# Kang-ChangWoo/audio-depth-estimation

Hardware: AMD Instinct MI355X
Metric: depth-maps/sec (train step) (higher is better)
Workload: dtype bf16; 1 GPU; unetbaseline_model unet_256 (ngf 64) train step, BatVisionV2-shaped 256x256, batch 32/GPU, Combined L1+SIlog loss, clip 1.0, AdamW; global_batch=32, image_size=256, launch=hipGraph, parallelism=dp1

## Files before the change

### audio-depth-estimation_amd/_lib.py

```python
from __future__ import annotations

import ctypes as C
import os

_HERE = os.path.dirname(os.path.abspath(__file__))
LIB_PATH = os.environ.get('ADN_LIB', os.path.join(_HERE, 'libadn.so'))

ADN_F32, ADN_BF16 = 0, 1
GEMM_S2, GEMM_T2, GEMM_S1 = 0, 1, 2
EPI_RAW, EPI_Z_STATS, EPI_ACT, EPI_BWD, EPI_FINAL, EPI_ADD = 0, 1, 2, 3, 4, 5

c_void_p, c_int32, c_int64, c_float = C.c_void_p, C.c_int32, C.c_int64, C.c_float


class AdnEpiSeg(C.Structure):
    _fields_ = [
        ('out0', c_void_p), ('out1', c_void_p), ('ref', c_void_p), ('z', c_void_p),
        ('mean', c_void_p), ('istd', c_void_p), ('scale', c_void_p), ('shift', c_void_p),
        ('bias', c_void_p), ('partials', c_void_p),
        ('channels', c_int32), ('slope', c_float), ('accumulate', c_int32), ('final_act', c_int32),
    ]


class AdnIgemmDesc(C.Structure):
    _fields_ = [
        ('dtype', c_int32), ('geom', c_int32), ('B', c_int32), ('Hs', c_int32), ('Ws', c_int32),
        ('C0', c_int32), ('C1', c_int32), ('N', c_int32),
        ('in0', c_void_p), ('in1', c_void_p), ('w', c_void_p),
        ('epi', c_int32), ('seg', AdnEpiSeg * 2),
        ('workspace', c_void_p), ('workspace_bytes', c_int64),
        ('ks', c_int32), ('reserved', c_int32),
    ]


class AdnMx8ConvDesc(C.Structure):
    _fields_ = [
        ('B', c_int32), ('H', c_int32), ('W', c_int32), ('C0', c_int32), ('C1', c_int32), ('N', c_int32),
        ('in0', c_void_p), ('sc0', c_void_p), ('in1', c_void_p), ('sc1', c_void_p), ('w', c_void_p), ('wsc', c_void_p),
        ('epi', c_int32), ('reserved', c_int32), ('seg', AdnEpiSeg * 2),
    ]


class AdnWgradDesc(C.Structure):
    _fields_ = [
        ('dtype', c_int32), ('B', c_int32), ('Hs', c_int32), ('Ws', c_int32),
        ('plain0', c_void_p), ('plain1', c_void_p), ('R0', c_int32), ('R1', c_int32),
        ('gath0', c_void_p), ('gath1', c_void_p), ('C0', c_int32), ('C1', c_int32),
        ('dw', c_void_p), ('workspace', c_void_p), ('workspace_bytes', c_int64), ('c_valid', c_int32),
        ('geom', c_int32), ('ks', c_int32), ('sq_partials', c_void_p),
    ]


class AdnAttnDesc(C.Structure):
    _fields_ = [
        ('dtype', c_int32), ('B2', c_int32), ('N', c_int32), ('dqk', c_int32), ('dv', c_int32), ('kv_shift', c_int32),
        ('q', c_void_p), ('k', c_void_p), ('v', c_void_p),
        ('ld_q', c_int32), ('ld_k', c_int32), ('ld_v', c_int32),
        ('o', c_void_p), ('ld_o', c_int32),
        ('lse', c_void_p), ('scale', c_float),
        ('dout', c_void_p), ('ld_do', c_int32),
        ('dq', c_void_p), ('dk', c_void_p), ('dvp', c_void_p),
        ('ld_dq', c_int32), ('ld_dk', c_int32), ('ld_dv', c_int32),
        ('workspace', c_void_p), ('workspace_bytes', c_int64),
    ]


class AdnDistillSmall(C.Structure):
    _fields_ = [
        ('mean_student', c_void_p), ('mean_teacher', c_void_p), ('centers_student', c_void_p), ('centers_teacher', c_void_p),
        ('feat_stats', c_void_p * 5), ('feat_channels', c_int32 * 5),
        ('pix_stats', c_void_p),
        ('B', c_int32), ('nb', c_int32), ('has_teacher', c_int32),
        ('temperature', c_float), ('lambda_task', c_float), ('lambda_response', c_float), ('lambda_feature', c_float),
        ('lambda_bin', c_float), ('lambda_sparse', c_float),
        ('terms', c_void_p), ('dmean', c_void_p), ('dcent', c_void_p),
    ]


class AdnCoarseLoss(C.Structure):
    _fields_ = [
        ('logits', c_void_p), ('dtype', c_int32), ('nb', c_int32), ('ld', c_int32), ('ce_mode', c_int32),
        ('pixels', c_int64), ('pixels_global', c_int64),
        ('centers', c_void_p), ('bins', c_void_p), ('gt', c_void_p), ('n_valid', c_void_p),
        ('sigma', c_float), ('gamma', c_float), ('ce_weight', c_float), ('reg_weight', c_float),
        ('depth', c_void_p), ('argmax', c_void_p), ('dlogits', c_void_p),
        ('workspace', c_void_p), ('workspace_bytes', c_int64),
    ]


class AdnDualRegLoss(C.Structure):
    _fields_ = [
        ('coarse', c_void_p), ('offset', c_void_p), ('gt', c_void_p), ('n_valid', c_void_p),
        ('pixels', c_int64), ('pixels_global', c_int64),
        ('coarse_weight', c_float), ('final_weight', c_float), ('offset_reg_weight', c_float),
        ('final_depth', c_void_p), ('dcoarse', c_void_p), ('doffset', c_void_p),
        ('workspace', c_void_p), ('workspace_bytes', c_int64),
    ]


class AdnHybridLoss(C.Structure):
    _fields_ = [
        ('logits', c_void_p), ('dtype', c_int32), ('nb', c_int32), ('ld', c_int32), ('reg_mode', c_int32),
        ('pixels', c_int64), ('pixels_global', c_int64),
        ('centers', c_void_p), ('coarse', c_void_p), ('offset', c_void_p), ('bins', c_void_p), ('gt', c_void_p),
        ('ce_weight', c_float), ('reg_weight', c_float), ('offset_reg_weight', c_float), ('label_smoothing', c_float),
        ('final_depth', c_void_p), ('dlogits', c_void_p), ('doffset', c_void_p),
        ('workspace', c_void_p), ('workspace_bytes', c_int64),
    ]


_PROTOS = {
    'adn_last_error': (C.c_char_p, []),
    'adn_version': (C.c_int, []),
    'adn_debug_poison_lds': (C.c_int, [c_void_p]),
    'adn_debug_stream_rmw': (C.c_int, [c_void_p, c_void_p, c_int64, c_int32, c_int32, c_void_p]),
    'adn_igemm_num_partials': (c_int64, [C.POINTER(AdnIgemmDesc)]),
    'adn_igemm_workspace_bytes': (c_int64, [C.POINTER(AdnIgemmDesc)]),
    'adn_igemm_describe': (C.c_int, [C.POINTER(AdnIgemmDesc), C.c_char_p, C.c_int]),
    'adn_igemm': (C.c_int, [C.POINTER(AdnIgemmDesc), c_void_p]),
    'adn_wgrad_workspace_bytes': (c_int64, [C.POINTER(AdnWgradDesc)]),
    'adn_wgrad': (C.c_int, [C.POINTER(AdnWgradDesc), c_void_p]),
    'adn_wgrad_batchable': (c_int32, [C.POINTER(AdnWgradDesc)]),
    'adn_wgrad_batch_sq_count': (c_int32, [C.POINTER(AdnWgradDesc)]),
    'adn_wgrad_batch': (C.c_int, [C.POINTER(AdnWgradDesc), c_int32, c_void_p]),
    'adn_wgrad_multi': (C.c_int, [C.POINTER(AdnWgradDesc), c_int32, c_void_p]),
    'adn_wgrad_patch_batch_workspace_bytes': (c_int64, [C.POINTER(AdnWgradDesc), c_int32]),
    'adn_wgrad_patch_batch': (C.c_int, [C.POINTER(AdnWgradDesc), c_int32, c_void_p]),
    'adn_wgrad_sq_count': (c_int32, [C.POINTER(AdnWgradDesc)]),
    'adn_pack_weights': (C.c_int, [c_void_p, c_int32, c_int32, c_int32, c_int32, c_void_p, c_void_p, c_void_p]),
    'adn_mx8_quantize': (C.c_int, [c_void_p, c_int64, c_int32, c_void_p, c_void_p, c_void_p]),
    'adn_mx8_pack': (C.c_int, [c_void_p, c_int32, c_int32, c_int32, c_void_p, c_void_p, c_void_p]),
    'adn_bn_partials_reduce': (C.c_int, [c_void_p, c_int64, c_int32, c_int32, c_void_p, c_void_p]),
    'adn_tail_stats_blocks': (c_int64, [c_int64, c_int32]),
    'adn_maxpool2_bwd_tail': (C.c_int, [c_void_p, c_void_p, c_void_p, c_int32, c_int32, c_int32, c_int32, c_int32, c_int32, c_void_p,
                                        c_void_p, c_void_p, c_void_p, c_void_p]),
    'adn_upsample2x_bwd_tail': (C.c_int, [c_void_p, c_void_p, c_int32, c_int32, c_int32, c_int32, c_int32, c_int32, c_int32, c_int32,
                                          c_void_p, c_void_p, c_void_p, c_void_p, c_void_p, c_void_p]),
    'adn_maxpool2_fwd_mx8': (C.c_int, [c_void_p, c_void_p, c_int32, c_int32, c_int32, c_int32, c_void_p, c_void_p, c_void_p]),
    'adn_upsample2x_fwd_mx8': (C.c_int, [c_void_p, c_void_p, c_int32, c_int32, c_int32, c_int32, c_int32, c_int32, c_void_p,
                                         c_void_p, c_void_p]),
    'adn_bn_act_mx8': (C.c_int, [c_void_p, c_int64, c_int32, c_void_p, c_void_p, c_void_p, c_void_p, c_void_p, c_void_p]),
    'adn_bn_bwd_apply_mx8': (C.c_int, [c_void_p, c_void_p, c_int64, c_int32, c_void_p, c_void_p, c_void_p, c_void_p, c_void_p,
                                       c_void_p, c_void_p]),
    'adn_conv3x3_mx8_num_partials': (c_int64, [C.POINTER(AdnMx8ConvDesc)]),
    'adn_conv3x3_mx8': (C.c_int, [C.POINTER(AdnMx8ConvDesc), c_void_p]),
    'adn_pack_rows': (C.c_int, [c_void_p, c_int32, c_int32, c_int32, c_int32, c_int32, c_int32, c_void_p, c_void_p]),
    'adn_pack_transpose_taps': (C.c_int, [c_void_p, c_int32, c_int32, c_int32, c_int32, c_int32, c_int32, c_void_p,
                                          c_void_p]),
    'adn_maxpool2_fwd': (C.c_int, [c_void_p, c_void_p, c_int32, c_int32, c_int32, c_int32, c_int32, c_void_p]),
    'adn_maxpool2_bwd': (C.c_int, [c_void_p, c_void_p, c_void_p, c_int32, c_int32, c_int32, c_int32, c_int32, c_int32, c_void_p]),
    'adn_upsample2x_fwd': (C.c_int, [c_void_p, c_void_p, c_int32, c_int32, c_int32, c_int32, c_int32, c_int32, c_int32, c_void_p]),
    'adn_upsample2x_bwd': (C.c_int, [c_void_p, c_void_p, c_int32, c_int32, c_int32, c_int32, c_int32, c_int32, c_int32, c_int32, c_void_p]),
    'adn_pixel_shuffle2': (C.c_int, [c_void_p, c_void_p, c_int32, c_int32, c_int32, c_int32, c_int32, c_int32, c_void_p]),
    'adn_relu_bwd_stats_num_partials': (c_int64, [c_int64, c_int32]),
    'adn_relu_bwd_stats': (C.c_int, [c_void_p, c_void_p, c_void_p, c_void_p, c_void_p, c_int64, c_int32, c_int32, c_void_p, c_void_p]),
    'adn_head1x1_fwd': (C.c_int, [c_void_p, c_void_p, c_void_p, c_int64, c_int32, c_int32, c_int32, c_float, c_void_p, c_void_p, c_void_p]),
    'adn_head1x1_bwd_workspace_bytes': (c_int64, [c_int64, c_int32]),
    'adn_head1x1_bwd': (C.c_int, [c_void_p, c_void_p, c_void_p, c_void_p, c_int64, c_int32, c_int32, c_int32, c_float, c_void_p, c_void_p, c_void_p, c_void_p,
                                  c_int64, c_void_p]),
    'adn_l1tv_workspace_bytes': (c_int64, [c_int64]),
    'adn_l1tv_stats': (C.c_int, [c_void_p, c_void_p, c_int32, c_int32, c_int32, c_void_p, c_void_p, c_int64, c_void_p]),
    'adn_l1tv_finish': (C.c_int, [c_void_p, c_void_p, c_int32, c_int32, c_int32, c_void_p, c_int32, c_float, c_float, c_void_p, c_void_p, c_void_p]),
    'adn_nchw_to_nhwc': (C.c_int, [c_void_p, c_void_p, c_int32, c_int32, c_int32, c_int32, c_int32, c_int32,
                                   c_void_p]),
    'adn_nchw_slice_to_nhwc': (C.c_int, [c_void_p, c_void_p, c_int32, c_int32, c_int32, c_int32, c_int32, c_int32, c_int32, c_int32, c_void_p]),
    'adn_attn_fwd': (C.c_int, [C.POINTER(AdnAttnDesc), c_void_p]),
    'adn_attn_bwd_workspace_bytes': (c_int64, [C.POINTER(AdnAttnDesc)]),
    'adn_attn_bwd': (C.c_int, [C.POINTER(AdnAttnDesc), c_void_p]),
    'adn_attn_form': (C.c_int, [C.POINTER(AdnAttnDesc), c_int32]),
    'adn_channel_sum_workspace_bytes': (c_int64, [c_int64, c_int32]),
    'adn_channel_sum': (C.c_int, [c_void_p, c_int64, c_int32, c_int32, c_int32, c_void_p, c_void_p, c_int64, c_void_p]),
    'adn_gate_bwd': (C.c_int, [c_void_p, c_void_p, c_int64, c_int32, c_void_p, c_void_p, c_void_p, c_int32, c_void_p, c_void_p, c_void_p, c_int64, c_void_p, c_int64,
# ... 191 lines not shown
```

### audio-depth-estimation_amd/engine.py

```python
from __future__ import annotations

import os

import torch

from . import _lib
from . import kernels as K
from .flat import FlatParamEngine
from ._lib import EPI_ACT, EPI_BWD, EPI_FINAL, EPI_RAW, EPI_Z_STATS, GEMM_S2, GEMM_T2

BN_EPS = 1e-5
BN_MOMENTUM = 0.1
LEAKY = 0.2


class UNetEngine(FlatParamEngine):

    def __init__(self, module, num_downs, depth_norm, compute_dtype=torch.bfloat16):
        self.module = module
        self.n = num_downs
        self.depth_norm = bool(depth_norm)
        self.dtype = compute_dtype
        self.levels = module._adn_levels()
        assert len(self.levels) == num_downs
# ... 116 lines not shown
                    pshape_d[i] = (hs, wsz, cd_out, 0, cd_in_p, 0)
                if cu_out_p == cu_out and K.wgrad_patch_batch_workspace_bytes(T, B, [(hs, wsz, c_up0, c_up1, cu_out_p, 0)]) >= 0:
                    pshape_u[i] = (hs, wsz, c_up0, c_up1, cu_out_p, 0)
            batching = T == torch.bfloat16 and not os.environ.get('ADN_NO_WGRAD_BATCH')
            lv['wb_d'], lv['wbq_d'] = (K.wgrad_batchable(T, B, hs, wsz, cd_out, 0, cd_in_p, 0)
                                       if batching and not edge0 and cd_in_p == cd_in else (0, 0))
            lv['wb_u'], lv['wbq_u'] = (K.wgrad_batchable(T, B, hs, wsz, c_up0, c_up1, cu_out_p, 0)
                                       if batching and not edge0 and cu_out_p == cu_out else (0, 0))
            for tag, bn, C in (('d', lv['bn_d'], cd_out), ('u', lv['bn_u'], cu_out)):
                if bn is None:
                    continue
                for nm in ('mean', 'istd', 'scale', 'shift'):
                    lv[f'{nm}_{tag}'] = torch.empty(C, **f32)
                lv[f'coef_{tag}'] = torch.empty(2 * C, **f32)
                lv[f'part_{tag}'] = torch.empty((pd if tag == 'd' else pu) * 2 * C, **f32)
        for i, lv in enumerate(self.levels):
            if lv['bn_u'] is not None:
                lv['bpart_u'] = torch.empty(self.levels[i - 1]['P_gu'] * 2 * lv['cu_out'], **f32)
            if lv['bn_d'] is not None:
                lv['bpart_d'] = torch.empty(self.levels[i + 1]['P_gd'] * 2 * lv['cd_out'], **f32)
        rows, t2_off, blk = [], 0, 0
        for lv in self.levels:
            for wk in ('down', 'up'):
                w = lv[wk].weight
                X, Y = w.shape[0], w.shape[1]
                rows.append([self.offset[id(w)], X, Y, t2_off, blk])
                lv[wk + '_t2_off'] = t2_off
                t2_off += 16 * X * Y
                blk += ((X + 63) // 64) * ((Y + 63) // 64) * 16
        self.t2_all = torch.empty(t2_off, dtype=T, device=dev)
        for lv in self.levels:
            for wk in ('down', 'up'):
                w = lv[wk].weight
                o = lv[wk + '_t2_off']
                lv[wk + '_t2'] = self.t2_all[o:o + 16 * w.shape[0] * w.shape[1]]
        def group(shapes):
            idx = sorted(shapes)[:4]
            ok = len(idx) >= 2 and idx == list(range(idx[0], idx[0] + len(idx)))
            return idx if ok else []
        self.pb_d, self.pb_u = group(pshape_d), group(pshape_u)
        self.pshape = {('d', i): pshape_d[i] for i in self.pb_d}
        self.pshape.update({('u', i): pshape_u[i] for i in self.pb_u})
        for tag, idx in (('d', self.pb_d), ('u', self.pb_u)):
            if idx:
                ws_bytes = max(ws_bytes, K.wgrad_patch_batch_workspace_bytes(T, B, [self.pshape[(tag, i)] for i in idx]))
        self._prepare_fused_norm(B, dev)
        if self.vae is not None:
            self._prepare_vae(B, dev)
        self.t2_table = torch.tensor(rows, dtype=torch.int64, device=dev)
        self.t2_layers, self.t2_blocks = len(rows), blk
        self.workspace = torch.empty(ws_bytes // 4 + 4, **f32)
        self.red_ws = torch.empty(4096, dtype=torch.float64, device=dev)
        self.weights_dirty = True
        self._shape_key = key
        self.B = B

    def _vae_level(self, i):
        return self.vae is not None and i == self.n - 1

    def _no_skip(self, i):
        return self.vae is not None and i == self.n - 2

    def _up_inputs(self, i):
        L = self.levels
        if self._no_skip(i):
            return L[i + 1]['ru'], None
        return L[i]['skip'], (L[i + 1]['ru'] if i < self.n - 1 else None)

    def _skip_relu(self, i):
        return i == 0 and self.skip0_leaky

    supports_fused_norm = True
    NORM_ROW = 8192

    def _prepare_fused_norm(self, B, dev):
        T = self.dtype
        self.sq_all = self.norm_ranges = None
        if os.environ.get('ADN_NO_FUSED_NORM'):
            return
        counts, covered = [], set()
        for i, lv in enumerate(self.levels):
            edge0 = i == 0 and self.edge_path
            hs, wsz = lv['hs'], lv['ws']
            c_up0, c_up1 = lv['cd_out'], lv['cu_in'] - lv['cd_out']
            nd = 0 if edge0 else K.wgrad_sq_count(T, B, hs, wsz, lv['cd_out'], 0, lv['down_ypad'], 0,
                                                  lv['cd_in'] if lv['down_ypad'] != lv['cd_in'] else 0)
            nu = 0 if edge0 else K.wgrad_sq_count(T, B, hs, wsz, c_up0, c_up1, lv['up_ypad'], 0,
                                                  lv['cu_out'] if lv['up_ypad'] != lv['cu_out'] else 0)
            if lv['wb_d']:
                nd = lv['wbq_d']
            if lv['wb_u']:
                nu = lv['wbq_u']
            for wk, cnt in (('down', nd), ('up', nu)):
                counts.append((lv, wk, cnt))
                if cnt:
                    covered.add(id(lv[wk].weight))
        rows = []
        for p, off, numel in self.param_meta:
            if id(p) in covered:
                continue
            for o in range(0, numel, self.NORM_ROW):
                rows.append([off + o, (min(self.NORM_ROW, numel - o) + 3) // 4 * 4])
        if not covered or len(rows) > 1024:
            return
        self.sq_all = torch.zeros(sum(c for _, _, c in counts), dtype=torch.float64, device=dev)
        o = 0
        for lv, wk, cnt in counts:
            lv[wk + '_sq'] = self.sq_all[o:o + cnt] if cnt else None
            o += cnt
        self.norm_ranges = torch.tensor(rows, dtype=torch.int64, device=dev).view(-1, 2) if rows else None

    def forward(self, x, training):
        if not x.is_cuda:
            raise RuntimeError('UnetGenerator.forward needs a HIP device tensor (libadn has no CPU path)')
        x = x.contiguous().float()
        self._prepare(x)
        if self.weights_dirty or self._packed_version != self._version_sum():
            self._pack_weights()
        T, B, n, L, ws = self.dtype, self.B, self.n, self.levels, self.workspace
        if self.edge_path:
            self._x_in, self._x_ver = x, x._version
        else:
            K.nchw_to_nhwc(x, self.x_nhwc)
        for i, lv in enumerate(L):
            src = self.x_nhwc if i == 0 else L[i - 1]['ad']
            C, hs, wsz = lv['cd_out'], lv['hs'], lv['ws']
            bn = lv['bn_d']
            if self._vae_level(i):
                K.igemm(T, GEMM_S2, B, hs, wsz, src, None, lv['down_s2'], C, EPI_RAW, [K.Seg(C, out0=self.vae_h)], ws)
                self._vae_forward(training)
            elif i == 0 and self.edge_path:
                K.l0_forward(x, self._flat_slice(self.flat_p, lv['down'].weight), B, hs, wsz, LEAKY, lv['ad'], lv['rd'])
            elif bn is None:
                K.igemm(T, GEMM_S2, B, hs, wsz, src, None, lv['down_s2'], C, EPI_ACT,
                        [K.Seg(C, out0=lv['ad'], out1=lv['rd'], slope=LEAKY)], ws, algo_c=lv['cd_in'])
            elif training:
                K.igemm(T, GEMM_S2, B, hs, wsz, src, None, lv['down_s2'], C, EPI_Z_STATS,
                        [K.Seg(C, out0=lv['zd'], partials=lv['part_d'])], ws)
                self._bn_forward(lv, 'd', bn, B * hs * wsz, lv['P_d'], lv['zd'], LEAKY, lv['ad'], lv['rd'])
            else:
                K.bn_eval_affine(bn.weight, bn.bias, bn.running_mean, bn.running_var, BN_EPS, lv['scale_d'],
                                 lv['shift_d'])
                K.igemm(T, GEMM_S2, B, hs, wsz, src, None, lv['down_s2'], C, EPI_ACT,
                        [K.Seg(C, out0=lv['ad'], out1=lv['rd'], scale=lv['scale_d'], shift=lv['shift_d'],
                               slope=LEAKY)], ws)
        for i in reversed(range(n)):
            lv = L[i]
            in0, in1 = self._up_inputs(i)
            C, hs, wsz = lv['cu_out'], lv['hs'], lv['ws']
            bn = lv['bn_u']
            if i == 0:
                bias = lv['up'].bias
                fa = self.final_act
                if self.n1_path:
                    K.convt_n1_forward(T, B, hs, wsz, in0, in1, self._flat_slice(self.flat_p, lv['up'].weight), bias,
                                       fa, lv['out'], ws, relu_in0=self._skip_relu(i))
                else:
                    K.igemm(T, GEMM_T2, B, hs, wsz, in0, in1, lv['up_t2'], C, EPI_FINAL,
                            [K.Seg(C, out0=lv['out'], bias=bias, final_act=fa)], ws)
            elif training:
                K.igemm(T, GEMM_T2, B, hs, wsz, in0, in1, lv['up_t2'], C, EPI_Z_STATS,
                        [K.Seg(C, out0=lv['zu'], partials=lv['part_u'])], ws)
                self._bn_forward(lv, 'u', bn, B * 4 * hs * wsz, lv['P_u'], lv['zu'], 0.0, None, lv['ru'])
            else:
                K.bn_eval_affine(bn.weight, bn.bias, bn.running_mean, bn.running_var, BN_EPS, lv['scale_u'],
                                 lv['shift_u'])
                K.igemm(T, GEMM_T2, B, hs, wsz, in0, in1, lv['up_t2'], C, EPI_ACT,
                        [K.Seg(C, out1=lv['ru'], scale=lv['scale_u'], shift=lv['shift_u'])], ws)
        out = L[0]['out']
        Cout = L[0]['cu_out']
        if Cout == 1:
            return out.view(B, 1, out.shape[1], out.shape[2])
        res = torch.empty(B, Cout, out.shape[1], out.shape[2], dtype=torch.float32, device=out.device)
        K.nhwc_to_nchw(out, res)
        return res

    BN_FUSED_MAX = int(os.environ.get('ADN_BN_FUSED_MAX', 1 << 20))

    def _bn_forward(self, lv, tag, bn, count, P, z, slope, out_leaky, out_relu):
        track = bn.track_running_stats and bn.running_mean is not None
        C = lv[f'mean_{tag}'].numel()
        args = (lv[f'part_{tag}'], P, C, count, bn.weight, bn.bias, BN_EPS,
                BN_MOMENTUM if bn.momentum is None else bn.momentum,
                bn.running_mean if track else None, bn.running_var if track else None,
                bn.num_batches_tracked if track else None,
                lv[f'mean_{tag}'], lv[f'istd_{tag}'], lv[f'scale_{tag}'], lv[f'shift_{tag}'])
        if count * C <= self.BN_FUSED_MAX and C % 32 == 0:
            K.bn_fwd_fused(*args, z, count, slope, out_leaky, out_relu)
        else:
            K.bn_fwd_finalize(*args)
            K.bn_act(z, count, C, lv[f'scale_{tag}'], lv[f'shift_{tag}'], slope, out_leaky, out_relu)

    def _bn_backward(self, lv, tag, bn, count, P, g, z):
        C = lv[f'mean_{tag}'].numel()
        dg, db = self._flat_slice(self.flat_g, bn.weight), self._flat_slice(self.flat_g, bn.bias)
        if count * C <= self.BN_FUSED_MAX and C % 32 == 0:
            K.bn_bwd_fused(lv[f'bpart_{tag}'], P, C, count, dg, db, g, z, count, lv[f'scale_{tag}'], lv[f'mean_{tag}'],
                           lv[f'istd_{tag}'])
        else:
            K.bn_bwd_finalize(lv[f'bpart_{tag}'], P, C, count, dg, db, lv[f'coef_{tag}'])
            K.bn_bwd_apply(g, z, count, C, lv[f'scale_{tag}'], lv[f'mean_{tag}'], lv[f'istd_{tag}'], lv[f'coef_{tag}'])

    def _ready(self, param):
        if self.on_grad_ready is not None:
            off = self.offset[id(param)]
            _lib.record_py(lambda: self.on_grad_ready(off))

    def dz_target(self):
        l0 = self.levels[0]
        if not getattr(self, 'edge_path', False) or l0.get('cu_out') != 1 or os.environ.get('ADN_NO_FUSED_DZ'):
            return None
        bias = l0['up'].bias
        return l0['dz0'], (None if bias is None else self._flat_slice(self.flat_g, bias)), self.final_act

    def backward(self, gout, fused_norm=False, dz_ready=False):
        T, B, n, L, ws = self.dtype, self.B, self.n, self.levels, self.workspace
        fused_norm = fused_norm and self.sq_all is not None
        l0 = L[0]
        if l0['cu_out'] != 1:
            raise NotImplementedError('backward is implemented for output_nc == 1 (the depth map)')
        up0 = l0['up']
        if not dz_ready:
            gout = gout.contiguous().float()
            K.final_act_bwd(gout, l0['out'], self.final_act, l0['dz0'])
            if up0.bias is not None:
                K.sum_to_scalar(l0['dz0'], self._flat_slice(self.flat_g, up0.bias), self.red_ws)
        batch = []
        held_u, held_d = [], []
# ... 122 lines not shown
```

### audio-depth-estimation_amd/kernels.py

```python
from __future__ import annotations

import ctypes as C
import os

import torch

from . import _lib
from ._lib import AdnAttnDesc, AdnCoarseLoss, AdnDistillSmall, AdnDualRegLoss, AdnHybridLoss
from ._lib import (ADN_BF16, ADN_F32, EPI_ACT, EPI_ADD, EPI_BWD, EPI_FINAL, EPI_RAW, EPI_Z_STATS, GEMM_S1, GEMM_S2, GEMM_T2,
                   AdnEpiSeg, AdnIgemmDesc, AdnMx8ConvDesc, AdnWgradDesc, ptr)

__all__ = ['dtype_code', 'Seg', 'igemm', 'igemm_query', 'wgrad', 'wgrad_workspace_bytes', 'pack_weights',
           'nchw_to_nhwc', 'nhwc_to_nchw', 'bn_fwd_finalize', 'bn_eval_affine', 'bn_act', 'bn_bwd_finalize',
           'bn_bwd_apply', 'loss_stats', 'loss_finish', 'final_act_bwd', 'sum_to_scalar', 'grad_norm', 'grad_norm_ranges', 'wgrad_sq_count',
           'optimizer_step', 'compute_errors', 'frontend', 'convt_n1_forward', 'convt_n1_workspace_bytes', 'vae_fwd',
           'vae_bwd', 'vae_bwd_workspace_bytes']


def _stream():
    return C.c_void_p(torch.cuda.current_stream().cuda_stream)


PROFILE = None


def _prof_begin():
    if PROFILE is None:
        return None
    ev = torch.cuda.Event(enable_timing=True)
    ev.record()
    return ev


def _prof_end(ev0, label, flops):
    if ev0 is None:
        return
    ev1 = torch.cuda.Event(enable_timing=True)
    ev1.record()
    PROFILE.append((label, flops, ev0, ev1))


def dtype_code(dt: torch.dtype) -> int:
    if dt == torch.float32:
        return ADN_F32
    if dt == torch.bfloat16:
        return ADN_BF16
    raise TypeError(f'libadn supports float32 and bfloat16 activations, got {dt}')


def _dev(*tensors):
    for t in tensors:
        if t is not None and not t.is_cuda:
            raise RuntimeError('libadn kernels need CUDA/HIP device tensors (no CPU fallback)')


class Seg:

    def __init__(self, channels, out0=None, out1=None, ref=None, z=None, mean=None, istd=None, scale=None,
                 shift=None, bias=None, partials=None, slope=0.0, accumulate=False, final_act=0):
        self.channels = channels
        self.tensors = (out0, out1, ref, z, mean, istd, scale, shift, bias, partials)
        self.slope, self.accumulate, self.final_act = slope, accumulate, final_act

    def fill(self, s: AdnEpiSeg):
        _dev(*self.tensors)
        (s.out0, s.out1, s.ref, s.z, s.mean, s.istd, s.scale, s.shift, s.bias, s.partials) = [ptr(t) for t in
                                                                                                 self.tensors]
        s.channels = self.channels
        s.slope = float(self.slope)
        s.accumulate = int(bool(self.accumulate))
        s.final_act = int(self.final_act)


def _igemm_desc(dtype, geom, B, Hs, Ws, in0, in1, w, N, epi, segs, workspace=None, ks=0):
    d = AdnIgemmDesc()
    d.ks = ks
    d.dtype, d.geom, d.B, d.Hs, d.Ws = dtype_code(dtype), geom, B, Hs, Ws
    d.C0 = in0.shape[-1]
    d.C1 = in1.shape[-1] if in1 is not None else 0
    d.N = N
    _dev(in0, in1, w, workspace)
    d.in0, d.in1, d.w = ptr(in0), ptr(in1), ptr(w)
    d.epi = epi
    segs[0].fill(d.seg[0])
    if len(segs) > 1:
        segs[1].fill(d.seg[1])
    d.workspace = ptr(workspace)
    d.workspace_bytes = workspace.numel() * workspace.element_size() if workspace is not None else 0
    return d


def igemm_query(dtype, geom, B, Hs, Ws, C0, C1, N, seg_channels, ks=0, epi=EPI_RAW):
    d = AdnIgemmDesc()
    d.ks = ks
    d.dtype, d.geom, d.B, d.Hs, d.Ws, d.C0, d.C1, d.N = dtype_code(dtype), geom, B, Hs, Ws, C0, C1, N
    d.in0 = d.w = 1
    d.in1 = 1 if C1 else None
    d.epi = epi
    d.seg[0].channels = seg_channels[0]
    d.seg[0].out0 = d.seg[0].ref = 1
    d.seg[1].channels = seg_channels[1] if len(seg_channels) > 1 else 0
    d.seg[1].out0 = d.seg[1].ref = 1
    lib = _lib.load()
    p = lib.adn_igemm_num_partials(C.byref(d))
    wsb = lib.adn_igemm_workspace_bytes(C.byref(d))
    if p < 0 or wsb < 0:
        raise RuntimeError('adn_igemm query failed: ' + lib.adn_last_error().decode())
    return p, wsb


def igemm(dtype, geom, B, Hs, Ws, in0, in1, w, N, epi, segs, workspace=None, algo_c=None, ks=0):
    d = _igemm_desc(dtype, geom, B, Hs, Ws, in0, in1, w, N, epi, segs, workspace, ks)
    ev = _prof_begin()
    _lib.call('adn_igemm', C.byref(d), _stream())
    flops = 2.0 * B * Hs * Ws * N * (ks * ks if geom == GEMM_S1 else 16) * (algo_c if algo_c else d.C0 + d.C1)
    _lib.annotate(label='igemm', flops=flops)
    if ev is not None:
        _prof_end(ev, 'igemm', flops)


def _wgrad_desc(dtype, B, Hs, Ws, plain0, plain1, gath0, gath1, dw, workspace, c_valid=0, ks=0):
    d = AdnWgradDesc()
    d.c_valid = c_valid
    d.geom, d.ks = (GEMM_S1, ks) if ks else (0, 0)
    d.dtype, d.B, d.Hs, d.Ws = dtype_code(dtype), B, Hs, Ws
    _dev(plain0, plain1, gath0, gath1, dw, workspace)
    d.plain0, d.plain1 = ptr(plain0), ptr(plain1)
    d.R0 = plain0.shape[-1]
    d.R1 = plain1.shape[-1] if plain1 is not None else 0
    d.gath0, d.gath1 = ptr(gath0), ptr(gath1)
    d.C0 = gath0.shape[-1]
    d.C1 = gath1.shape[-1] if gath1 is not None else 0
    d.dw = ptr(dw)
    d.workspace = ptr(workspace)
    d.workspace_bytes = workspace.numel() * workspace.element_size() if workspace is not None else 0
    return d


def wgrad_workspace_bytes(dtype, B, Hs, Ws, R0, R1, C0, C1, c_valid=0, ks=0):
    d = AdnWgradDesc()
    d.c_valid = c_valid
    d.geom, d.ks = (GEMM_S1, ks) if ks else (0, 0)
    d.dtype, d.B, d.Hs, d.Ws, d.R0, d.R1, d.C0, d.C1 = dtype_code(dtype), B, Hs, Ws, R0, R1, C0, C1
    d.plain0 = d.gath0 = d.dw = 1
    d.plain1 = 1 if R1 else None
    d.gath1 = 1 if C1 else None
    lib = _lib.load()
    n = lib.adn_wgrad_workspace_bytes(C.byref(d))
    if n < 0:
        raise RuntimeError('adn_wgrad query failed: ' + lib.adn_last_error().decode())
    return n


def wgrad_batchable(dtype, B, Hs, Ws, R0, R1, C0, C1, c_valid=0):
    d = AdnWgradDesc()
    d.c_valid = c_valid
    d.geom, d.ks = 0, 0
    d.dtype, d.B, d.Hs, d.Ws, d.R0, d.R1, d.C0, d.C1 = dtype_code(dtype), B, Hs, Ws, R0, R1, C0, C1
    d.plain0 = d.gath0 = d.dw = 1
    d.plain1 = 1 if R1 else None
    d.gath1 = 1 if C1 else None
    lib = _lib.load()
    return int(lib.adn_wgrad_batchable(C.byref(d))), int(lib.adn_wgrad_batch_sq_count(C.byref(d)))


def wgrad_batch(dtype, B, problems, entry='adn_wgrad_batch'):
    arr = (AdnWgradDesc * len(problems))()
    flops = 0.0
# ... 919 lines not shown
```

### include/adn.h

```cpp
#ifndef ADN_H_
#define ADN_H_

#include <stdint.h>

#ifdef __cplusplus
extern "C" {
#endif

#define ADN_OK 0
#define ADN_ERR_ARG (-1)
#define ADN_ERR_LAUNCH (-2)
#define ADN_ERR_UNSUPPORTED (-3)

enum { ADN_F32 = 0, ADN_BF16 = 1 };

enum {
  ADN_GEMM_S2 = 0,
  ADN_GEMM_T2 = 1,
  ADN_GEMM_S1 = 2
};

enum {
  ADN_EPI_RAW = 0,
  ADN_EPI_Z_STATS,
  ADN_EPI_ACT,
  ADN_EPI_BWD,
  ADN_EPI_FINAL,
  ADN_EPI_ADD
};

typedef struct {
  void* out0;
  void* out1;
  const void* ref;
  const void* z;
  const float* mean;
  const float* istd;
  const float* scale;
  const float* shift;
  const float* bias;
  float* partials;
  int32_t channels;
  float slope;
  int32_t accumulate;
  int32_t final_act;
} AdnEpiSeg;

typedef struct {
  int32_t dtype;
  int32_t geom;
  int32_t B;
  int32_t Hs, Ws;
  int32_t C0, C1;
  int32_t N;
  const void* in0;
  const void* in1;
  const void* w;
  int32_t epi;
  AdnEpiSeg seg[2];
  void* workspace;
  int64_t workspace_bytes;
  int32_t ks;
  int32_t reserved;
} AdnIgemmDesc;

const char* adn_last_error(void);
int adn_version(void);
int adn_debug_poison_lds(void* stream);
int adn_debug_stream_rmw(const void* src, void* dst, int64_t bytes, int32_t workgroups, int32_t passes, void* stream);

int64_t adn_igemm_num_partials(const AdnIgemmDesc* d);
int64_t adn_igemm_workspace_bytes(const AdnIgemmDesc* d);
int adn_igemm_describe(const AdnIgemmDesc* d, char* buf, int len);

int adn_igemm(const AdnIgemmDesc* d, void* stream);

typedef struct {
  int32_t dtype;
  int32_t B, Hs, Ws;
  const void* plain0; const void* plain1; int32_t R0, R1;
  const void* gath0;  const void* gath1;  int32_t C0, C1;
  float* dw;
  void* workspace; int64_t workspace_bytes;
  int32_t c_valid;
  int32_t geom;
  int32_t ks;
  double* sq_partials;
} AdnWgradDesc;
int64_t adn_wgrad_workspace_bytes(const AdnWgradDesc* d);
int adn_wgrad(const AdnWgradDesc* d, void* stream);
int32_t adn_wgrad_batchable(const AdnWgradDesc* d);
int32_t adn_wgrad_batch_sq_count(const AdnWgradDesc* d);
int adn_wgrad_batch(const AdnWgradDesc* descs, int32_t n, void* stream);
int adn_wgrad_multi(const AdnWgradDesc* descs, int32_t n, void* stream);
int64_t adn_wgrad_patch_batch_workspace_bytes(const AdnWgradDesc* descs, int32_t n);
int adn_wgrad_patch_batch(const AdnWgradDesc* descs, int32_t n, void* stream);
int32_t adn_wgrad_sq_count(const AdnWgradDesc* d);

int adn_pack_weights(const float* master, int32_t X, int32_t Y, int32_t y_pad, int32_t dtype,
                     void* s2_out, void* t2_out, void* stream);

int adn_pack_rows(const float* master, int32_t X, int32_t taps, int32_t Y, int32_t y_pad,
                  int32_t row_stride, int32_t dtype, void* out, void* stream);
int adn_pack_transpose_taps(const float* master, int32_t X, int32_t taps, int32_t Y, int32_t flip,
                            int32_t row_stride, int32_t dtype, void* out, void* stream);

int adn_mx8_quantize(const void* src_bf16, int64_t rows, int32_t C, void* dst_e4m3, void* scales_e8m0, void* stream);
int adn_mx8_pack(const float* master, int32_t X, int32_t Y, int32_t transpose, void* w8, void* wsc, void* stream);
int adn_bn_act_mx8(const void* z, int64_t pixels, int32_t C, const float* scale, const float* shift, void* out_relu,
                   void* out8, void* out_scales, void* stream);
int adn_bn_bwd_apply_mx8(void* g, const void* z, int64_t pixels, int32_t C, const float* scale, const float* mean,
                         const float* istd, const float* coef, void* out8, void* out_scales, void* stream);
int adn_maxpool2_fwd_mx8(const void* src, void* dst, int32_t B, int32_t H, int32_t W, int32_t C, void* out8,
                         void* out_scales, void* stream);
int adn_upsample2x_fwd_mx8(const void* src, void* dst, int32_t B, int32_t Hi, int32_t Wi, int32_t Ho, int32_t Wo,
                           int32_t C, void* out8, void* out_scales, void* stream);
typedef struct {
  int32_t B, H, W;
  int32_t C0, C1, N;
  const void* in0;
  const void* sc0;
  const void* in1;
  const void* sc1;
  const void* w;
  const void* wsc;
  int32_t epi;
  int32_t reserved;
  AdnEpiSeg seg[2];
// ... 304 lines not shown
```

Baseline: 12550 depth-maps/s.

## Add skinny stride-2 conv kernel with fused BatchNorm stats for tiny-grid levels

Adds a dedicated HIP kernel for the deep U-Net down-convolutions whose output grid is at most 2x2 with at most 128 rows. Each workgroup owns 16 output channels, splits the taps across four waves, and streams channel chunks through a 4-stage LDS ring using buffer loads. Because each workgroup sees every row, it reduces BatchNorm statistics in-kernel and applies the affine plus leaky/ReLU outputs and running-stat updates in the same launch, replacing the igemm + partials + BN finalize + apply sequence. The aim is to cut launch count and to expose channel parallelism on these tiny-M layers. The cost is a large new kernel that must match the existing numerics, and it launches only N/16 workgroups.

```diff
diff --git a/audio-depth-estimation_amd/_lib.py b/audio-depth-estimation_amd/_lib.py
--- a/audio-depth-estimation_amd/_lib.py
+++ b/audio-depth-estimation_amd/_lib.py
@@ -30,6 +30,15 @@
         ('epi', c_int32), ('seg', AdnEpiSeg * 2),
         ('workspace', c_void_p), ('workspace_bytes', c_int64),
         ('ks', c_int32), ('reserved', c_int32),
+    ]
+
+
+class AdnSkinnyBn(C.Structure):
+    _fields_ = [
+        ('gamma', c_void_p), ('beta', c_void_p), ('eps', c_float), ('momentum', c_float),
+        ('running_mean', c_void_p), ('running_var', c_void_p), ('num_batches_tracked', c_void_p),
+        ('mean', c_void_p), ('istd', c_void_p), ('scale', c_void_p), ('shift', c_void_p),
+        ('out_leaky', c_void_p), ('out_relu', c_void_p), ('slope', c_float), ('reserved', c_int32),
     ]
 
 
@@ -118,6 +127,7 @@
     'adn_igemm_workspace_bytes': (c_int64, [C.POINTER(AdnIgemmDesc)]),
     'adn_igemm_describe': (C.c_int, [C.POINTER(AdnIgemmDesc), C.c_char_p, C.c_int]),
     'adn_igemm': (C.c_int, [C.POINTER(AdnIgemmDesc), c_void_p]),
+    'adn_igemm_skinny': (C.c_int, [C.POINTER(AdnIgemmDesc), C.POINTER(AdnSkinnyBn), c_void_p]),
     'adn_wgrad_workspace_bytes': (c_int64, [C.POINTER(AdnWgradDesc)]),
     'adn_wgrad': (C.c_int, [C.POINTER(AdnWgradDesc), c_void_p]),
     'adn_wgrad_batchable': (c_int32, [C.POINTER(AdnWgradDesc)]),
diff --git a/audio-depth-estimation_amd/csrc/igemm_skinny.hip b/audio-depth-estimation_amd/csrc/igemm_skinny.hip
--- /dev/null
+++ b/audio-depth-estimation_amd/csrc/igemm_skinny.hip
@@ -0,0 +1,349 @@
+#include <type_traits>
+
+#include "epilogue.h"
+
+namespace {
+
+constexpr int SK_NW = 4;
+constexpr int SK_CK = 32;
+constexpr int SK_MAXM = 128;
+[[maybe_unused]] constexpr int SK_MAXT = SK_MAXM / 16;
+constexpr int SK_STAGES = 4;
+
+struct SkinnyParams {
+  const uint16_t* in0;
+  const uint16_t* w;
+  int B, Hs, Ws, C, N, M;
+  int epi;
+  AdnEpiSeg seg;
+  AdnSkinnyBn bn;
+};
+
+template <int N>
+__device__ __forceinline__ void sk_wait_vmcnt() {
+  asm volatile("s_waitcnt vmcnt(%0) lgkmcnt(0)" ::"n"(N) : "memory");
+}
+
+__device__ __forceinline__ int sk_swz(int b) { return (0x1320 >> (((b >> 2) & 3) << 2)) & 3; }
+
+template <int HS, int WS, int TPB>
+__global__ __launch_bounds__(SK_NW * 64) void igemm_skinny_s2_kernel(SkinnyParams p) {
+#if defined(__HIP_DEVICE_COMPILE__)
+  constexpr int NPOSS = HS * WS, NT = NPOSS * TPB;
+  static_assert(NT <= SK_MAXT, "at most 128 rows");
+  constexpr int NJ = NT;
+  constexpr int NTY = HS == 1 ? 1 : 2, NTX = WS == 1 ? 1 : 2;
+  constexpr int NTAP = NTY * NTX;
+  constexpr int STAGE_BYTES = SK_NW * NJ * 1024;
+  constexpr int PER_CHUNK = NTAP + NJ;
+  constexpr unsigned OOB = 0x80000000u;
+  typedef __attribute__((address_space(3))) void* lptr_t;
+  extern __shared__ __attribute__((aligned(16))) char smem[];
+  const int tid = threadIdx.x, lane = tid & 63;
+  const int wave = __builtin_amdgcn_readfirstlane(tid >> 6);
+  const int frow = lane & 15, fq = lane >> 4;
+  const int n0 = blockIdx.x * 16;
+  const int B = p.B, C = p.C, M = p.M;
+  constexpr int Hs = HS, Ws = WS, Wl = 2 * WS, npos = 4 * HS * WS, tpb = TPB, ntiles = NT, Mpad = NT * 16;
+  const int npix = B * npos;
+  const int kyh = wave >> 1, kxh = wave & 1;
+  auto tap_ky = [&](int a) { return HS == 1 ? 1 + kyh : (kyh ? 3 - a : a); };
+  auto tap_kx = [&](int c) { return WS == 1 ? 1 + kxh : (kxh ? 3 - c : c); };
+  auto pos_y = [&](int ly) { return (HS == 2 && kyh) ? 1 - ly : ly; };
+  auto pos_x = [&](int lx) { return (WS == 2 && kxh) ? 1 - lx : lx; };
+
+  int abase[NT];
+#pragma unroll
+  for (int t = 0; t < NT; ++t) {
+    const int lp = t / TPB, bt = t % TPB;
+    const int y = pos_y(lp / WS), x = pos_x(lp % WS);
+    int b = bt * 16 + frow;
+    b = b < B ? b : 0;
+    abase[t] = ((2 * y * Wl + 2 * x) * B + b) * 64 + ((fq ^ sk_swz(b)) << 4);
+  }
+  int tapshift[NTAP], tapk[NTAP];
+#pragma unroll
+  for (int a = 0; a < NTY; ++a)
+#pragma unroll
+    for (int c = 0; c < NTX; ++c) {
+      const int ky = tap_ky(a), kx = tap_kx(c);
+      tapshift[a * NTX + c] = ((ky - 1) * Wl + (kx - 1)) * B * 64;
+      tapk[a * NTX + c] = ((n0 * 16 + ky * 4 + kx) * C) * 2;
+    }
+
+  unsigned dvoff[NJ];
+#pragma unroll
+  for (int k = 0; k < NJ; ++k) {
+    const int pi = 16 * (wave * NJ + k) + (lane >> 2);
+    const int pos = pi / B, b = pi - pos * B;
+    const int q = (lane & 3) ^ sk_swz(b);
+    dvoff[k] = pi < npix ? (unsigned)(((b * npos + pos) * C + q * 8) * 2) : OOB;
+  }
+  const int w_voff = (frow * 16 * C + fq * 8) * 2;
+  const __amdgpu_buffer_rsrc_t rs_in = __builtin_amdgcn_make_buffer_rsrc((void*)p.in0, 0, npix * C * 2, 0x00020000);
+  const __amdgpu_buffer_rsrc_t rs_w = __builtin_amdgcn_make_buffer_rsrc((void*)p.w, 0, p.N * 16 * C * 2, 0x00020000);
+
+  const int nch = C / SK_CK;
+  u32x4_t wr[SK_STAGES][NTAP];
+  f32x4_t acc[NT];
+#pragma unroll
+  for (int t = 0; t < NT; ++t) acc[t] = f32x4_t{0.f, 0.f, 0.f, 0.f};
+
+#define SK_ISSUE(ch, st)                                                                                              \
+  do {                                                                                                                \
+    asm volatile("" ::: "memory");                                                                                    \
+    const int c0b_ = (ch) * SK_CK * 2;                                                                                \
+    _Pragma("unroll") for (int k_ = 0; k_ < NTAP; ++k_)                                                               \
+        wr[st][k_] = __builtin_amdgcn_raw_buffer_load_b128(rs_w, w_voff, tapk[k_] + c0b_, 0);                         \
+    _Pragma("unroll") for (int k_ = 0; k_ < NJ; ++k_)                                                                 \
+        __builtin_amdgcn_raw_ptr_buffer_load_lds(rs_in, (lptr_t)(smem + (st) * STAGE_BYTES + (wave * NJ + k_) * 1024), \
+                                                 16, dvoff[k_], c0b_, 0, 0);                                          \
+    asm volatile("" ::: "memory");                                                                                    \
+  } while (0)
+
+  auto inside = [](int k, int t) {
+    const int a = k / NTX, c = k % NTX, lp = t / TPB;
+    return (HS == 1 || a == 1 || lp / WS == 1) && (WS == 1 || c == 1 || lp % WS == 1);
+  };
+  auto step = [&](int i, auto U, auto STEADY) {
+    constexpr int u = decltype(U)::value;
+    constexpr bool steady = decltype(STEADY)::value;
+    if (steady || i + 2 < nch) sk_wait_vmcnt<2 * PER_CHUNK>();
+    else sk_wait_vmcnt<0>();
+    __builtin_amdgcn_s_barrier();
+    asm volatile("" ::: "memory");
+    if (steady || i + SK_STAGES - 1 < nch) SK_ISSUE(i + SK_STAGES - 1, (u + SK_STAGES - 1) % SK_STAGES);
+    const char* stage = smem + u * STAGE_BYTES;
+    u32x4_t af[NTAP][NT];
+#pragma unroll
+    for (int k = 0; k < NTAP; ++k)
+#pragma unroll
+      for (int t = 0; t < NT; ++t)
+        if (inside(k, t)) af[k][t] = *reinterpret_cast<const u32x4_t*>(stage + abase[t] + tapshift[k]);
+#pragma unroll
+    for (int k = 0; k < NTAP; ++k)
+#pragma unroll
+      for (int t = 0; t < NT; ++t)
+        if (inside(k, t)) mma_tile<uint16_t>(af[k][t], wr[u][k], acc[t]);
+  };
+  using std::integral_constant;
+  int i0 = 0;
+  if (nch >= 2 * SK_STAGES - 1) {
+    SK_ISSUE(0, 0);
+    SK_ISSUE(1, 1);
+    SK_ISSUE(2, 2);
+    for (; i0 + 2 * SK_STAGES - 1 <= nch; i0 += SK_STAGES) {
+      step(i0 + 0, integral_constant<int, 0>{}, integral_constant<bool, true>{});
+      step(i0 + 1, integral_constant<int, 1>{}, integral_constant<bool, true>{});
+      step(i0 + 2, integral_constant<int, 2>{}, integral_constant<bool, true>{});
+      step(i0 + 3, integral_constant<int, 3>{}, integral_constant<bool, true>{});
+    }
+  } else {
+#pragma unroll
+    for (int s = 0; s < SK_STAGES - 1; ++s)
+      if (s < nch) SK_ISSUE(s, s);
+  }
+  for (; i0 < nch; i0 += SK_STAGES) {
+    step(i0 + 0, integral_constant<int, 0>{}, integral_constant<bool, false>{});
+    if (i0 + 1 < nch) step(i0 + 1, integral_constant<int, 1>{}, integral_constant<bool, false>{});
+    if (i0 + 2 < nch) step(i0 + 2, integral_constant<int, 2>{}, integral_constant<bool, false>{});
+    if (i0 + 3 < nch) step(i0 + 3, integral_constant<int, 3>{}, integral_constant<bool, false>{});
+  }
+#undef SK_ISSUE
+
+  __syncthreads();
+  float* red = reinterpret_cast<float*>(smem);
+#pragma unroll
+  for (int t = 0; t < NT; ++t) {
+    const int lp = t / TPB;
+    const int at = (pos_y(lp / WS) * WS + pos_x(lp % WS)) * TPB + t % TPB;
+#pragma unroll
+    for (int r = 0; r < 4; ++r) red[(wave * Mpad + at * 16 + 4 * fq + r) * 16 + frow] = acc[t][r];
+  }
+  __syncthreads();
+
+  const int rr = tid >> 1, cg = tid & 1;
+  const int et = rr >> 4;
+  const int epos = et / tpb, eb = (et - epos * tpb) * 16 + (rr & 15);
+  const bool rowok = et < ntiles && eb < B;
+  const int nl = n0 + cg * 8;
+  const int64_t op = (int64_t)eb * (Hs * Ws) + epos;
+  float v[8];
+#pragma unroll
+  for (int e = 0; e < 8; ++e) v[e] = 0.f;
+  if (rowok) {
+    f32x4_t s0 = *reinterpret_cast<const f32x4_t*>(red + rr * 16 + cg * 8);
+    f32x4_t s1 = *reinterpret_cast<const f32x4_t*>(red + rr * 16 + cg * 8 + 4);
+#pragma unroll
+    for (int w = 1; w < SK_NW; ++w) {
+      const f32x4_t a0 = *reinterpret_cast<const f32x4_t*>(red + (w * Mpad + rr) * 16 + cg * 8);
+      const f32x4_t a1 = *reinterpret_cast<const f32x4_t*>(red + (w * Mpad + rr) * 16 + cg * 8 + 4);
+#pragma unroll
+      for (int e = 0; e < 4; ++e) {
+        s0[e] += a0[e];
+        s1[e] += a1[e];
+      }
+    }
+#pragma unroll
+    for (int e = 0; e < 4; ++e) {
+      v[e] = s0[e];
+      v[4 + e] = s1[e];
+    }
+  }
+  const AdnEpiSeg& sg = p.seg;
+
+  if (p.epi == ADN_EPI_ACT) {
+    if (rowok) {
+      float d1[8], d2[8];
+      EpiCols cols;
+      epi_cols_init<uint16_t>(ADN_EPI_ACT, sg, nl, cols);
+      epi_vec8<uint16_t>(ADN_EPI_ACT, sg, cols, op, nl, v, d1, d2);
+    }
+    return;
+  }
+
+  float* zt = red + SK_NW * Mpad * 16;
+  double* dpart = reinterpret_cast<double*>(zt + Mpad * 16);
+  float* aff = reinterpret_cast<float*>(dpart + 2 * 8 * 16);
+  float zb[8];
+#pragma unroll
+  for (int e = 0; e < 8; ++e) zb[e] = 0.f;
+  if (rowok) {
+#pragma unroll
+    for (int e = 0; e < 8; ++e) zb[e] = v[e] + (sg.bias ? sg.bias[nl + e] : 0.f);
+    store8<uint16_t>(sg.out0, op * sg.channels + nl, zb);
+  }
+  if (rr < Mpad) {
+#pragma unroll
+    for (int e = 0; e < 8; ++e) zt[rr * 16 + cg * 8 + e] = zb[e];
+  }
+  __syncthreads();
+  {
+    const int st = tid >> 7, c = (tid >> 3) & 15, rg = tid & 7;
+    double s = 0.0;
+    for (int r = rg; r < Mpad; r += 8) {
+      const float z = zt[r * 16 + c];
+      s += st ? (double)(z * z) : (double)z;
+    }
+    dpart[(st * 8 + rg) * 16 + c] = s;
+  }
+  __syncthreads();
+  if (tid < 16) {
+    double s1 = 0.0, s2 = 0.0;
+#pragma unroll
+    for (int g = 0; g < 8; ++g) {
+      s1 += dpart[g * 16 + tid];
+      s2 += dpart[(8 + g) * 16 + tid];
+    }
+    const int c = n0 + tid;
+    const double count = (double)M;
+    const double mu = s1 / count;
+    double var = s2 / count - mu * mu;
+    if (var < 0.0) var = 0.0;
+    const double is = 1.0 / sqrt(var + (double)p.bn.eps);
+    const double g = p.bn.gamma ? (double)p.bn.gamma[c] : 1.0, bt = p.bn.beta ? (double)p.bn.beta[c] : 0.0;
+    const float sc = (float)(g * is), shf = (float)(bt - mu * g * is);
+    aff[tid] = sc;
+    aff[16 + tid] = shf;
+    p.bn.mean[c] = (float)mu;
+    p.bn.istd[c] = (float)is;
+    p.bn.scale[c] = sc;
+    p.bn.shift[c] = shf;
+    if (p.bn.running_mean) {
+      const float momentum = p.bn.momentum;
+      const double unbiased = count > 1.0 ? var * count / (count - 1.0) : var;
+      p.bn.running_mean[c] = (float)((1.0 - momentum) * (double)p.bn.running_mean[c] + momentum * mu);
+      p.bn.running_var[c] = (float)((1.0 - momentum) * (double)p.bn.running_var[c] + momentum * unbiased);
+    }
+    if (p.bn.num_batches_tracked && c == 0) p.bn.num_batches_tracked[0] += 1;
+  }
+  __syncthreads();
+  if (rowok) {
+    const int64_t e0 = op * sg.channels + nl;
+    const float slope = p.bn.slope;
+    float y[8], o[8];
+#pragma unroll
+    for (int k = 0; k < 8; ++k) {
+      const float zr = bf16_bits_to_f32(f32_to_bf16_bits(zb[k]));
+      y[k] = zr * aff[cg * 8 + k] + aff[16 + cg * 8 + k];
+    }
+    if (p.bn.out_leaky) {
+#pragma unroll
+      for (int k = 0; k < 8; ++k) o[k] = y[k] > 0.f ? y[k] : y[k] * slope;
+      store8<uint16_t>(p.bn.out_leaky, e0, o);
+    }
+    if (p.bn.out_relu) {
+#pragma unroll
+      for (int k = 0; k < 8; ++k) o[k] = fmaxf(y[k], 0.f);
+      store8<uint16_t>(p.bn.out_relu, e0, o);
+    }
+  }
+#endif
+}
+
+template <int HS, int WS, int TPB>
+int launch_skinny(const SkinnyParams& p, hipStream_t st) {
+  if constexpr (HS * WS * TPB > SK_MAXT) {
+    return ADN_ERR_ARG;
+  } else {
+    constexpr int mpad = HS * WS * TPB * 16;
+    constexpr int fin_bytes = (SK_NW + 1) * mpad * 16 * 4 + 2 * 8 * 16 * 8 + 2 * 16 * 4;
+    constexpr int ring_bytes = SK_STAGES * SK_NW * (HS * WS * TPB) * 1024;
+    constexpr int lds = ring_bytes > fin_bytes ? ring_bytes : fin_bytes;
+    static_assert(lds <= 160 * 1024, "LDS budget");
+    ADN_SET_LDS_ONCE(160 * 1024, &igemm_skinny_s2_kernel<HS, WS, TPB>);
+    hipLaunchKernelGGL((igemm_skinny_s2_kernel<HS, WS, TPB>), dim3(p.N / 16), dim3(SK_NW * 64), lds, st, p);
+    ADN_CHECK_LAUNCH();
+    return ADN_OK;
+  }
+}
+
+template <int HS, int WS>
+int launch_skinny_tpb(const SkinnyParams& p, hipStream_t st) {
+  const int tiles = (p.B + 15) / 16;
+  if (tiles <= 1) return launch_skinny<HS, WS, 1>(p, st);
+  if (tiles <= 2) return launch_skinny<HS, WS, 2>(p, st);
+  if (tiles <= 4) return launch_skinny<HS, WS, 4>(p, st);
+  return launch_skinny<HS, WS, 8>(p, st);
+}
+
+}
+
+extern "C" int adn_igemm_skinny(const AdnIgemmDesc* d, const AdnSkinnyBn* bn, void* stream) {
+  ADN_CHECK_ARG(d != nullptr, "adn_igemm_skinny: null descriptor");
+  ADN_CHECK_ARG(d->dtype == ADN_BF16, "adn_igemm_skinny: bf16 only (dtype %d)", d->dtype);
+  ADN_CHECK_ARG(d->geom == ADN_GEMM_S2, "adn_igemm_skinny: geometry %d is not built (ADN_GEMM_S2 only)", d->geom);
+  ADN_CHECK_ARG(d->B > 0 && d->Hs > 0 && d->Ws > 0 && d->Hs <= 2 && d->Ws <= 2, "adn_igemm_skinny: small grid %d x %d, at most 2 x 2",
+                d->Hs, d->Ws);
+  const int64_t M = (int64_t)d->B * d->Hs * d->Ws;
+  ADN_CHECK_ARG(M <= SK_MAXM, "adn_igemm_skinny: M = %lld small-grid rows, at most %d", (long long)M, SK_MAXM);
+  ADN_CHECK_ARG(d->N > 0 && d->N % 16 == 0 && d->N <= 4096, "adn_igemm_skinny: N = %d must be a multiple of 16 (at most 4096)", d->N);
+  ADN_CHECK_ARG(d->C0 > 0 && d->C0 % SK_CK == 0 && d->C0 <= 4096 && d->C1 == 0,
+                "adn_igemm_skinny: C0 = %d must be a multiple of %d (at most 4096), C1 = %d must be 0", d->C0, SK_CK, d->C1);
+  ADN_CHECK_ARG(d->in0 && d->w, "adn_igemm_skinny: null operand");
+  ADN_CHECK_ARG(d->seg[0].channels == d->N && d->seg[1].channels == 0, "adn_igemm_skinny: one output segment of N channels");
+  ADN_CHECK_ARG(d->epi == ADN_EPI_ACT || d->epi == ADN_EPI_Z_STATS, "adn_igemm_skinny: epilogue %d is not built (ACT, Z_STATS)", d->epi);
+  if (d->epi == ADN_EPI_ACT) {
+    ADN_CHECK_ARG(bn == nullptr, "adn_igemm_skinny: ADN_EPI_ACT takes no BatchNorm block");
+    ADN_CHECK_ARG(d->seg[0].out0 || d->seg[0].out1, "adn_igemm_skinny: no output");
+  } else {
+    ADN_CHECK_ARG(bn != nullptr, "adn_igemm_skinny: ADN_EPI_Z_STATS needs the BatchNorm block");
+    ADN_CHECK_ARG(d->seg[0].out0 && bn->mean && bn->istd && bn->scale && bn->shift, "adn_igemm_skinny: null required pointer");
+    ADN_CHECK_ARG((bn->running_mean == nullptr) == (bn->running_var == nullptr), "adn_igemm_skinny: running stats mismatch");
+  }
+  SkinnyParams p = {};
+  p.in0 = reinterpret_cast<const uint16_t*>(d->in0);
+  p.w = reinterpret_cast<const uint16_t*>(d->w);
+  p.B = d->B;
+  p.Hs = d->Hs;
+  p.Ws = d->Ws;
+  p.C = d->C0;
+  p.N = d->N;
+  p.M = (int)M;
+  p.epi = d->epi;
+  p.seg = d->seg[0];
+  if (bn) p.bn = *bn;
+  hipStream_t st = reinterpret_cast<hipStream_t>(stream);
+  if (d->Hs == 1) return d->Ws == 1 ? launch_skinny_tpb<1, 1>(p, st) : launch_skinny_tpb<1, 2>(p, st);
+  return d->Ws == 1 ? launch_skinny_tpb<2, 1>(p, st) : launch_skinny_tpb<2, 2>(p, st);
+}
diff --git a/audio-depth-estimation_amd/engine.py b/audio-depth-estimation_amd/engine.py
--- a/audio-depth-estimation_amd/engine.py
+++ b/audio-depth-estimation_amd/engine.py
@@ -192,6 +192,7 @@
         self.workspace = torch.empty(ws_bytes // 4 + 4, **f32)
         self.red_ws = torch.empty(4096, dtype=torch.float64, device=dev)
         self.weights_dirty = True
+        self.skinny_layers = set()
         self._shape_key = key
         self.B = B
 
@@ -272,12 +273,20 @@
             elif i == 0 and self.edge_path:
                 K.l0_forward(x, self._flat_slice(self.flat_p, lv['down'].weight), B, hs, wsz, LEAKY, lv['ad'], lv['rd'])
             elif bn is None:
-                K.igemm(T, GEMM_S2, B, hs, wsz, src, None, lv['down_s2'], C, EPI_ACT,
-                        [K.Seg(C, out0=lv['ad'], out1=lv['rd'], slope=LEAKY)], ws, algo_c=lv['cd_in'])
+                if self._skinny(i, 'L', EPI_ACT, src.shape[-1], C):
+                    K.igemm_skinny(T, GEMM_S2, B, hs, wsz, src, None, lv['down_s2'], C, EPI_ACT,
+                                   K.Seg(C, out0=lv['ad'], out1=lv['rd'], slope=LEAKY), algo_c=lv['cd_in'])
+                else:
+                    K.igemm(T, GEMM_S2, B, hs, wsz, src, None, lv['down_s2'], C, EPI_ACT,
+                            [K.Seg(C, out0=lv['ad'], out1=lv['rd'], slope=LEAKY)], ws, algo_c=lv['cd_in'])
             elif training:
-                K.igemm(T, GEMM_S2, B, hs, wsz, src, None, lv['down_s2'], C, EPI_Z_STATS,
-                        [K.Seg(C, out0=lv['zd'], partials=lv['part_d'])], ws)
-                self._bn_forward(lv, 'd', bn, B * hs * wsz, lv['P_d'], lv['zd'], LEAKY, lv['ad'], lv['rd'])
+                if self._skinny(i, 'L', EPI_Z_STATS, src.shape[-1], C):
+                    K.igemm_skinny(T, GEMM_S2, B, hs, wsz, src, None, lv['down_s2'], C, EPI_Z_STATS, K.Seg(C, out0=lv['zd']),
+                                   self._skinny_bn(lv, 'd', bn, LEAKY, lv['ad'], lv['rd']))
+                else:
+                    K.igemm(T, GEMM_S2, B, hs, wsz, src, None, lv['down_s2'], C, EPI_Z_STATS,
+                            [K.Seg(C, out0=lv['zd'], partials=lv['part_d'])], ws)
+                    self._bn_forward(lv, 'd', bn, B * hs * wsz, lv['P_d'], lv['zd'], LEAKY, lv['ad'], lv['rd'])
             else:
                 K.bn_eval_affine(bn.weight, bn.bias, bn.running_mean, bn.running_var, BN_EPS, lv['scale_d'],
                                  lv['shift_d'])
@@ -314,6 +323,22 @@
         res = torch.empty(B, Cout, out.shape[1], out.shape[2], dtype=torch.float32, device=out.device)
         K.nhwc_to_nchw(out, res)
         return res
+
+    def _skinny(self, i, kind, epi, c_in, n):
+        lv = self.levels[i]
+        ok = (not os.environ.get('ADN_NO_SKINNY') and not self._vae_level(i)
+              and K.igemm_skinny_ok(self.dtype, GEMM_S2, self.B, lv['hs'], lv['ws'], c_in, 0, n, epi))
+        if ok:
+            self.skinny_layers.add(f'{kind}{i}')
+        return ok
+
+    def _skinny_bn(self, lv, tag, bn, slope, out_leaky, out_relu):
+        track = bn.track_running_stats and bn.running_mean is not None
+        return dict(gamma=bn.weight, beta=bn.bias, eps=BN_EPS, momentum=BN_MOMENTUM if bn.momentum is None else bn.momentum,
+                    running_mean=bn.running_mean if track else None, running_var=bn.running_var if track else None,
+                    num_batches_tracked=bn.num_batches_tracked if track else None,
+                    mean=lv[f'mean_{tag}'], istd=lv[f'istd_{tag}'], scale=lv[f'scale_{tag}'], shift=lv[f'shift_{tag}'],
+                    out_leaky=out_leaky, out_relu=out_relu, slope=slope)
 
     BN_FUSED_MAX = int(os.environ.get('ADN_BN_FUSED_MAX', 1 << 20))
 
diff --git a/audio-depth-estimation_amd/kernels.py b/audio-depth-estimation_amd/kernels.py
--- a/audio-depth-estimation_amd/kernels.py
+++ b/audio-depth-estimation_amd/kernels.py
@@ -8,9 +8,9 @@
 from . import _lib
 from ._lib import AdnAttnDesc, AdnCoarseLoss, AdnDistillSmall, AdnDualRegLoss, AdnHybridLoss
 from ._lib import (ADN_BF16, ADN_F32, EPI_ACT, EPI_ADD, EPI_BWD, EPI_FINAL, EPI_RAW, EPI_Z_STATS, GEMM_S1, GEMM_S2, GEMM_T2,
-                   AdnEpiSeg, AdnIgemmDesc, AdnMx8ConvDesc, AdnWgradDesc, ptr)
-
-__all__ = ['dtype_code', 'Seg', 'igemm', 'igemm_query', 'wgrad', 'wgrad_workspace_bytes', 'pack_weights',
+                   AdnEpiSeg, AdnIgemmDesc, AdnMx8ConvDesc, AdnSkinnyBn, AdnWgradDesc, ptr)
+
+__all__ = ['dtype_code', 'Seg', 'igemm', 'igemm_skinny', 'igemm_skinny_ok', 'igemm_query', 'wgrad', 'wgrad_workspace_bytes', 'pack_weights',
            'nchw_to_nhwc', 'nhwc_to_nchw', 'bn_fwd_finalize', 'bn_eval_affine', 'bn_act', 'bn_bwd_finalize',
            'bn_bwd_apply', 'loss_stats', 'loss_finish', 'final_act_bwd', 'sum_to_scalar', 'grad_norm', 'grad_norm_ranges', 'wgrad_sq_count',
            'optimizer_step', 'compute_errors', 'frontend', 'convt_n1_forward', 'convt_n1_workspace_bytes', 'vae_fwd',
@@ -114,6 +114,34 @@
     ev = _prof_begin()
     _lib.call('adn_igemm', C.byref(d), _stream())
     flops = 2.0 * B * Hs * Ws * N * (ks * ks if geom == GEMM_S1 else 16) * (algo_c if algo_c else d.C0 + d.C1)
+    _lib.annotate(label='igemm', flops=flops)
+    if ev is not None:
+        _prof_end(ev, 'igemm', flops)
+
+
+SKINNY_MAX_ROWS = 128
+
+
+def igemm_skinny_ok(dtype, geom, B, Hs, Ws, C0, C1, N, epi):
+    return (dtype == torch.bfloat16 and geom == GEMM_S2 and epi in (EPI_ACT, EPI_Z_STATS) and Hs <= 2 and Ws <= 2
+            and B * Hs * Ws <= SKINNY_MAX_ROWS and N % 16 == 0 and N <= 4096 and C0 % 32 == 0 and 0 < C0 <= 4096
+            and C1 == 0)
+
+
+def igemm_skinny(dtype, geom, B, Hs, Ws, in0, in1, w, N, epi, seg, bn=None, algo_c=None):
+    d = _igemm_desc(dtype, geom, B, Hs, Ws, in0, in1, w, N, epi, [seg])
+    blk = None
+    if bn is not None:
+        blk = AdnSkinnyBn()
+        tens = [bn.get(k) for k in ('gamma', 'beta', 'running_mean', 'running_var', 'num_batches_tracked', 'mean', 'istd',
+                                    'scale', 'shift', 'out_leaky', 'out_relu')]
+        _dev(*tens)
+        (blk.gamma, blk.beta, blk.running_mean, blk.running_var, blk.num_batches_tracked, blk.mean, blk.istd, blk.scale,
+         blk.shift, blk.out_leaky, blk.out_relu) = [ptr(t) for t in tens]
+        blk.eps, blk.momentum, blk.slope = float(bn['eps']), float(bn['momentum']), float(bn.get('slope', 0.0))
+    ev = _prof_begin()
+    _lib.call('adn_igemm_skinny', C.byref(d), C.byref(blk) if blk is not None else None, _stream())
+    flops = 2.0 * B * Hs * Ws * N * 16 * (algo_c if algo_c else d.C0 + d.C1)
     _lib.annotate(label='igemm', flops=flops)
     if ev is not None:
         _prof_end(ev, 'igemm', flops)
diff --git a/include/adn.h b/include/adn.h
--- a/include/adn.h
+++ b/include/adn.h
@@ -74,6 +74,24 @@
 int adn_igemm_describe(const AdnIgemmDesc* d, char* buf, int len);
 
 int adn_igemm(const AdnIgemmDesc* d, void* stream);
+
+typedef struct {
+  const float* gamma;
+  const float* beta;
+  float eps, momentum;
+  float* running_mean;
+  float* running_var;
+  int64_t* num_batches_tracked;
+  float* mean;
+  float* istd;
+  float* scale;
+  float* shift;
+  void* out_leaky;
+  void* out_relu;
+  float slope;
+  int32_t reserved;
+} AdnSkinnyBn;
+int adn_igemm_skinny(const AdnIgemmDesc* d, const AdnSkinnyBn* bn, void* stream);
 
 typedef struct {
   int32_t dtype;
```

Result: no change. 12540 depth-maps/s (median of 2 runs) (-0.1%).
